# zhangyi-3/UCDIR

Hardware: AMD Instinct MI355X
Metric: restored images/sec at 50-step p_sample_loop, 256x256 SID (higher is better)
Workload: dtype bf16

## Files before the change

### ucdir_amd/csrc/conv_sk.hip.h

```cpp
#pragma once
#include "conv_halo.hip.h"
#include "akgm_ws.hip.h"

struct ConvSkP {
    const bf16_t* A; long long a_par_stride;
    const bf16_t* B0; const bf16_t* B1; int c0, ld0, ld1;
    int nchunks;
    int nb, H, W, Wp, Hp;
    int ns, Ws, Wpe, HpWpe, npos;
    float inv_per_b, inv_HpWpe, inv_Wpe;
    int ntiles, rowtiles, npar;
    int nhp;
    int nfeat;
    float alpha; int fold; int act;
    const stat_t* stats0; const stat_t* stats1; double inv_count;
    const float* bias; const float* Tb; const float* Tg; int tab_ld;
    const bf16_t* res; int res_ld;
    bf16_t* out; int out_ld;
    stat_t* stats_out;
    int units, ndp;
    float* partial;
    int alt_units; const bf16_t* alt_A; const float* alt_bias; bf16_t* alt_out; int alt_out_ld;
    int mix_wt, mix_nt, mix_nhp, mix_nunits, mix_nndp, mix_q0, mix_srt;
    unsigned long long* dbg;
};

template <int MW, int NW = 8>
struct CvSk {
    static constexpr int NWN = NW / MW;
    static constexpr int NPX = 64 * NWN;
    static constexpr int ROWS = 128 * MW;
    static constexpr int STAGE = 8192 * MW;
    static constexpr int PW = 8 * MW / NW;
    static constexpr bool LDS_TAB = NW == 8;
    static constexpr int OFF_W = 0;
    static constexpr int OFF_TB = 4 * STAGE;
    static constexpr int OFF_TG = OFF_TB + (LDS_TAB ? 9 * ROWS * 4 : 0);
    static constexpr int OFF_MS = OFF_TG + (LDS_TAB ? 9 * ROWS * 4 : 0);
// ... 5 lines not shown
    static constexpr int LDS_MAX = NW == 8 ? 160 * 1024 : 80 * 1024;
    __host__ __device__ static constexpr int lds_bytes(int nhp) { return OFF_H + 2 * nhp * 1024; }
    __host__ __device__ static constexpr int part_floats() { return ROWS * NPX; }
};

#ifdef UCDIR_TIMING
#define SK_STAMP() do { if (dbg_on && dbg_n < 120) p.dbg[dbg_off + dbg_n++] = __builtin_amdgcn_s_memtime(); } while (0)
#else
#define SK_STAMP() do {} while (0)
#endif

__device__ __forceinline__ void sk_dma16(const void* sbase, unsigned voff, unsigned lds_dst) {
    asm volatile("s_mov_b32 m0, %2\n\ts_nop 0\n\tglobal_load_lds_dwordx4 %0, %1" :: "v"(voff), "s"(sbase), "s"(lds_dst) : "memory", "m0");
}

template <int N>
__device__ __forceinline__ void sk_wait_vm() { asm volatile("s_waitcnt vmcnt(%0)" :: "n"(N) : "memory"); }

struct SkSched {
    int units, ndp, nch, G;
    long long tc;
    __host__ __device__ SkSched(int units_, int ndp_, int nch_, int G_) : units(units_), ndp(ndp_), nch(nch_), G(G_), tc((long long)(units_ - ndp_) * nch_) {}
    __host__ __device__ long long start(int g) const { return tc * g / G; }
};

__device__ __forceinline__ int sk_udiv(int q, int d, float inv_d) {
    int t = (int)((float)q * inv_d);
    t = t * d > q ? t - 1 : t;
    t = (t + 1) * d <= q ? t + 1 : t;
    return t;
// ... 278 lines not shown
            float v[16];
#pragma unroll
            for (int g4 = 0; g4 < 4; ++g4) {
                f32x4_t bv = {0.f, 0.f, 0.f, 0.f};
                if (p.alt_bias) bv = *reinterpret_cast<const f32x4_t*>(p.alt_bias + fo + 4 * g4);
#pragma unroll
                for (int e = 0; e < 4; ++e) v[4 * g4 + e] = acc[f][n][4 * g4 + e] + bv[e];
            }
            bf16_t* op = p.alt_out + opos * p.alt_out_ld + fo;
            *reinterpret_cast<uint4*>(op) = pack8_bf16(v);
            *reinterpret_cast<uint4*>(op + 8) = pack8_bf16(v + 8);
        }
    }
}

template <int MW, int NW, int NTAPS, int NF = 4>
__device__ __forceinline__ void conv_sk_body(const ConvSkP& p, unsigned char* smem, const int lid, const int G, const int units_arg, const int ndp_arg,
                                             const int qbase, const int nhp) {
    using L = CvSk<MW, NW>;
    static_assert(NF == 4 || (NF == 2 && MW == 1 && NW == 4), "short units: four waves of 64 x 64");
    constexpr int PWN = L::PW * NF / 4;
    constexpr int RSUB = 4 / NF;
    constexpr int NWN = L::NWN;
    const int tid = threadIdx.x, lane = tid & 63, l31 = lane & 31, hh = lane >> 5;
    const int wave = __builtin_amdgcn_readfirstlane(tid >> 6);
    const int wm = wave / NWN, wn = wave % NWN;
#ifdef UCDIR_TIMING
    const bool dbg_on = p.dbg && (lid == G / 2 + 3 || lid == G - 3) && (lane == 0) && (wave == NW - 1);
    const int dbg_off = lid == G - 3 ? 128 : 0;
    int dbg_n = 0;
#endif
    SK_STAMP();
    const int Wp = p.Wpe, nch = p.nchunks;
    const int HB = nhp * 1024;
    constexpr int NHW = L::NHW;
    constexpr int TA = NTAPS - 3 > 1 ? NTAPS - 3 : 1;
    constexpr int HPER = (NHW + TA - 1) / TA;

    const unsigned a_lane = L::OFF_W + (NF == 4 ? (4 * wm) * 2048 : 0) + lane * 16;
    unsigned bx[NTAPS];
    auto set_bx = [&](int py, int pxp) {
#pragma unroll
        for (int t = 0; t < NTAPS; ++t) {
            int ky, kx;
            if (NTAPS == 9) { ky = t / 3; kx = t - 3 * ky; } else { ky = py + (t >> 1); kx = pxp + (t & 1); }
            const int hp = wn * 64 + l31 + ky * Wp + kx;
            bx[t] = L::OFF_H + (hp << 6) + (((hh ^ (hp >> 2)) & 3) << 4);
        }
    };
    if (NTAPS == 9) set_bx(0, 0);
    const int hpos0 = (lane >> 2) - Wp - 1;
    const unsigned hsw = (unsigned)(((lane & 3) ^ ((lane >> 4) & 3)) << 3);
    auto piece_of = [&](int j) { const int i = j * NW + wave; return i < nhp ? i : nhp - 1; };

    const SkSched sch(units_arg, ndp_arg, nch, G);
    const long long c_beg = sch.start(lid), c_end = sch.start(lid + 1);
    const int ndp_mine = lid < ndp_arg ? (ndp_arg - lid + G - 1) / G : 0;
    long long cpos = c_beg;
    int dpi = 0;
    struct Seg { int unit, cb, ce, par, rt, tile; bool first_sk, ok; };
// ... 25 lines not shown
        const bool first = ch < p.c0;
        const int ld = first ? p.ld0 : p.ld1;
        hsrc = first ? p.B0 + ch : p.B1 + (ch - p.c0);
        if (ld != ld_cur) {
#pragma unroll
            for (int j = 0; j < NHW; ++j) hq[j] = ((((hq[j] >> 1) - hsw) / (unsigned)ld_cur) * (unsigned)ld + hsw) * 2u;
            ld_cur = ld;
        }
    };
    const unsigned char* a_seg = nullptr;
    const unsigned lane16 = (unsigned)lane * 16u;
    int seg_cb = 0;
    auto issue_halo = [&](int j, int buf) {
        sk_dma16(hsrc, hq[j], (unsigned)(L::OFF_H + piece_of(j) * 1024 + buf * HB));
    };
    auto issue_stage = [&](int k, int slot) {
#pragma unroll
        for (int j = 0; j < PWN; ++j)
            sk_dma16(a_seg + (long long)k * L::STAGE + j * 1024, lane16, (unsigned)(L::OFF_W + slot * L::STAGE + (wave * PWN + j) * 1024));
    };
    constexpr int NTP = 10;
    auto issue_table = [&](int rt, int i, int buf) {
        const int seg = 2 * i + (lane >> 5);
        const float* src = reinterpret_cast<const float*>(p.A);
        if (seg == 0 || seg > 18) { if (p.bias) src = p.bias + rt * L::ROWS; }
        else if (seg < 10) { if (p.fold) src = p.Tb + (long long)(seg - 1) * p.tab_ld + rt * L::ROWS; }
        else if (p.fold) src = p.Tg + (long long)(seg - 10) * p.tab_ld + rt * L::ROWS;
        __builtin_amdgcn_global_load_lds((const GLOBAL_AS void*)(src + (lane & 31) * 4), (LDS_AS void*)(smem + L::OFF_H + buf * HB + i * 1024), 16, 0, 0);
    };
    int hb0 = 0;
    auto prefetch = [&](const Seg& s) {
        if (NTAPS != 9) set_bx(s.par >> 1, s.par & 1);
        const int q0 = qbase + s.tile * L::NPX;
#pragma unroll
        for (int j = 0; j < NHW; ++j) {
            int q = q0 + hpos0 + 16 * piece_of(j);
            q = q < 0 ? 0 : (q >= p.npos ? (q - p.npos < p.npos ? q - p.npos : 0) : q);
            int b, yp, xs, xp;
            sk_decode(p, q, b, yp, xs, xp);
            xp = xp < p.Wp ? xp : p.Wp - 1;
            hq[j] = (unsigned)((b * p.Hp + yp) * p.Wp + xp);
        }
        ld_cur = s.cb * 32 < p.c0 ? p.ld0 : p.ld1;
#pragma unroll
        for (int j = 0; j < NHW; ++j) hq[j] = (hq[j] * (unsigned)ld_cur + hsw) * 2u;
        halo_chunk(s.cb);
        a_seg = reinterpret_cast<const unsigned char*>(p.A + (long long)s.par * p.a_par_stride + ((long long)(s.rt / RSUB) * nch * NTAPS) * (L::STAGE / 2) +
                                                       (s.rt % RSUB) * (L::STAGE / 2 / RSUB) + (wave * PWN) * 512);
        seg_cb = s.cb;
#pragma unroll
        for (int j = 0; j < NHW; ++j) issue_halo(j, hb0);
#pragma unroll
        for (int k = 0; k < 4; ++k) issue_stage(s.cb * NTAPS + k, k);
    };

    Seg cur = next_segment();
    if (!cur.ok) return;
    int rt_cur = cur.rt;
    prefetch(cur);
    auto sample_range = [&](const Seg& s) {
        const int per_b = p.ns * p.HpWpe;
        const int b0 = sk_udiv(qbase + s.tile * L::NPX, per_b, p.inv_per_b);
        int b1 = sk_udiv(qbase + s.tile * L::NPX + L::NPX - 1, per_b, p.inv_per_b) + 1; b1 = b1 < p.nb ? b1 : p.nb;
        if (b0 < b1) sk_sample_table(p, reinterpret_cast<float*>(smem + L::OFF_MS) + 2 * b0, b0, b1, wave, NW, lane);
    };
    if (L::LDS_TAB) {
// ... 31 lines not shown
            const unsigned b0 = (bx[t] + boff) ^ (jj << 5);
            lds_read16_asm<0>(fb[jj][0], b0);
            lds_read16_asm<2048>(fb[jj][1], b0);
        };
        __builtin_amdgcn_sched_barrier(0);
        unsigned bcur = hb0 ? (unsigned)HB : 0u;
        reads(std::integral_constant<int, 0>{}, std::integral_constant<int, 0>{}, 0, bcur);
        reads(std::integral_constant<int, 0>{}, std::integral_constant<int, 1>{}, 0, bcur);

        int h = 0;
        const bool want_tab = !L::LDS_TAB && cb == 0 && ce == nch;
#pragma unroll 1
        for (int c = cb; c < ce; ++c) {
            const unsigned bnext = bcur ? 0u : (unsigned)HB;
            const int cn = c + 1 < ce ? c + 1 : c;
            halo_chunk(cn);
            static_for<0, NTAPS>([&](auto tc) {
                constexpr int t = decltype(tc)::value;
                constexpr int tn = (t + 1) % NTAPS;
                constexpr int tm1 = (t + NTAPS - 1) % NTAPS;
                const unsigned boffn = tn == 0 ? bnext : bcur;
                const unsigned aan = a_lane + (unsigned)(((h + 1) & 3) * L::STAGE);
                auto unit = [&](auto jc, auto&& shadow) {
                    constexpr int jj = decltype(jc)::value;
                    const unsigned b0 = (bx[tn] + boffn) ^ (jj << 5);
#define SK_MF(f, n) acc[f][n] = __builtin_amdgcn_mfma_f32_32x32x16_bf16(fa[jj][f], fb[jj][n], acc[f][n], 0, 0, 0); __builtin_amdgcn_sched_barrier(0)
                    if constexpr (NF == 2) {
                        SK_MF(0, 0); shadow(std::integral_constant<int, 0>{}); __builtin_amdgcn_sched_barrier(0);
                        SK_MF(1, 0); lds_read16_asm<0>(fb[jj][0], b0); shadow(std::integral_constant<int, 1>{}); __builtin_amdgcn_sched_barrier(0);
                        SK_MF(0, 1); lds_read16_asm<0 * 2048 + jj * 1024>(fa[jj][0], aan); shadow(std::integral_constant<int, 2>{}); __builtin_amdgcn_sched_barrier(0);
                        SK_MF(1, 1); lds_read16_asm<1 * 2048 + jj * 1024>(fa[jj][1], aan); lds_read16_asm<2048>(fb[jj][1], b0); __builtin_amdgcn_sched_barrier(0);
                    } else {
                    SK_MF(0, 0); shadow(std::integral_constant<int, 0>{}); __builtin_amdgcn_sched_barrier(0);
                    SK_MF(1, 0); shadow(std::integral_constant<int, 1>{}); __builtin_amdgcn_sched_barrier(0);
                    SK_MF(2, 0); shadow(std::integral_constant<int, 2>{}); __builtin_amdgcn_sched_barrier(0);
#ifdef SK_ABL_NOREAD
// ... 7 lines not shown
#endif
                    }
#undef SK_MF
                };
#ifndef SK_ABL_NOREAD
                lgkm_wait_asm<NF + 2>();
#endif
                unit(std::integral_constant<int, 0>{}, [&](auto) {});
#ifndef SK_ABL_NOREAD
                lgkm_wait_asm<NF + 2>();
#endif
                {
                    constexpr int j0p = tm1 * HPER < NHW ? tm1 * HPER : NHW, j1p = (tm1 + 1) * HPER < NHW ? (tm1 + 1) * HPER : NHW;
                    constexpr int c1 = tm1 < TA ? j1p - j0p : 0;
#ifndef SK_ABL_NODMA
                    sk_wait_vm<PWN + c1>();
#endif
#ifndef SK_ABL_NOBAR
                    asm volatile("s_barrier" ::: "memory");
#endif
                }
                unit(std::integral_constant<int, 1>{}, [&](auto sc) {
                    constexpr int sidx = decltype(sc)::value;
                    constexpr int j0 = t < TA ? (t * HPER < NHW ? t * HPER : NHW) : 0, j1 = t < TA ? ((t + 1) * HPER < NHW ? (t + 1) * HPER : NHW) : 0;
                    constexpr int nh = j1 - j0;
                    constexpr int total = nh + PWN;
                    static_for<0, total>([&](auto qc) {
                        constexpr int q = decltype(qc)::value;
#ifdef SK_ABL_NODMA
                        constexpr int sh = 99;
#else
                        constexpr int sh = q * 3 / total;
#endif
                        if constexpr (sh == sidx) {
                            if constexpr (q < nh) {
                                constexpr int j = j0 + q;
                                if (want_tab && c + 1 == ce && j * NW + wave < NTP) issue_table(cur.rt / RSUB, j * NW + wave, bnext ? 1 : 0);
                                else issue_halo(j, bnext ? 1 : 0);
                            } else {
                                constexpr int j = q - nh;
                                sk_dma16(a_seg + (long long)(cb * NTAPS + h + 4) * L::STAGE + j * 1024, lane16, (unsigned)(L::OFF_W + (h & 3) * L::STAGE + (wave * PWN + j) * 1024));
                            }
                        }
                    });
                });
                ++h;
            });
            bcur = bnext;
        }
        asm volatile("s_waitcnt vmcnt(0) lgkmcnt(0)" ::: "memory");
#pragma unroll
        for (int jj = 0; jj < 2; ++jj) {
#pragma unroll
            for (int f = 0; f < NF; ++f) asm volatile("" : "+v"(fa[jj][f]));
            asm volatile("" : "+v"(fb[jj][0]), "+v"(fb[jj][1]));
        }
        __builtin_amdgcn_sched_barrier(0);
        asm volatile("s_barrier" ::: "memory");
        SK_STAMP();
        const bool same_rt = nxt.ok && (nxt.rt == rt_cur || !L::LDS_TAB);
        const unsigned tab_base = (unsigned)L::OFF_H + bcur;
        hb0 = bcur ? 0 : 1;
        if (same_rt) prefetch(nxt);
        __builtin_amdgcn_sched_barrier(0);

        if (NF != 4 || (cb == 0 && ce == nch)) {
            sk_epilogue<MW, NW, L::LDS_TAB ? 1 : 2, true, NF>(p, smem, nullptr, acc, cur.par, cur.rt / RSUB, qbase + cur.tile * L::NPX, wm, wn, lane, tab_base, -1,
                                                             (cur.rt % RSUB) * (32 * NF));
        } else if constexpr (NF == 4) {
            float* pw = p.partial + ((long long)(2 * lid + (cur.first_sk ? 0 : 1))) * L::part_floats() + wave * (128 * 64) + lane * 4;
#pragma unroll
            for (int f = 0; f < 4; ++f)
#pragma unroll
                for (int n = 0; n < 2; ++n)
#pragma unroll
// ... 40 lines not shown
        }
        if (!mixed) {
            const int q = nblk >> 3, r = nblk & 7, xcd = bid & 7;
            lid = (xcd < r ? xcd * (q + 1) : r * (q + 1) + (xcd - r) * q) + (bid >> 3);
            G = nblk;
        }
        if (MW == 1 && NW == 4) {
            if (alt) {
                const int lane = threadIdx.x & 63, wave = __builtin_amdgcn_readfirstlane(threadIdx.x >> 6);
                sk_alt_unit<NW>(p, smem, lid, wave, lane);
                return;
            }
        }
    }
    conv_sk_body<MW, NW, NTAPS>(p, smem, lid, G, p.units, p.ndp, 0, p.nhp);
}

template <int MW, int NW>
__global__ __launch_bounds__(64) void conv_sk_finish_kernel(const ConvSkP p, int G) {
    using L = CvSk<MW, NW>;
    __shared__ float ms[2 * L::MAXB];
    constexpr int NWN = L::NWN;
    const int lane = threadIdx.x;
    const int wave = blockIdx.x >> 2, fsel = blockIdx.x & 3;
    const int wm = wave / NWN, wn = wave % NWN;
    const int nch = p.nchunks;
    const SkSched sch(p.units, p.ndp, nch, G);
    const int u = blockIdx.y;
    const long long a = (long long)u * nch, b = a + nch;
    int g = (int)(a * G / sch.tc);
// ... 64 lines not shown
```

### ucdir_amd/csrc/engine.hip

```cpp
#include <hip/hip_runtime.h>

#include <cmath>
#include <cstdio>
#include <cstring>
#include <map>
#include <mutex>
#include <set>
#include <array>
#include <atomic>
#include <memory>
#include <string>
#include <vector>

#include "../../include/ucdir_hip.h"
#include "cgemm.hip.h"
#include "conv_halo.hip.h"
#include "akgm_halo.hip.h"
#include "akgm_pre.hip.h"
#include "akgm_ws.hip.h"
#include "akgm_ws32.hip.h"
#include "akgm_ws64.hip.h"
#include "conv_ws.hip.h"
#include "conv_sk.hip.h"
#include "conv_ws128.hip.h"
// ... 62 lines not shown
    ~DevPool() { release(); }
};

struct ConvW {
    bf16_t* A = nullptr; float* bias = nullptr; float* Tb = nullptr; float* Tg = nullptr;
    int rows_pad = 0, Kpad = 0, ntaps = 0, cin = 0, cout = 0, TM = 128; bool fold = false;
    bf16_t* Aup = nullptr; int Kup = 0;
    bf16_t* A10 = nullptr; float* bias_res = nullptr;
    bf16_t* Aws = nullptr;
    bf16_t* Aws128 = nullptr;
    bf16_t* Aqkv = nullptr;
    bf16_t* Atile = nullptr;
    bf16_t* Ask[2] = {nullptr, nullptr}; bf16_t* Ask_up[2] = {nullptr, nullptr};
    long long sk_up_stride[2] = {0, 0};
    bf16_t* Ask1x1 = nullptr;
};
struct AkgmW {
    bf16_t* A = nullptr; float* bias = nullptr; float* Tb = nullptr; float* Tg = nullptr;
    float* Tbb = nullptr;
    bf16_t* Apre = nullptr;
    bf16_t* Aws32 = nullptr;
    bf16_t* Aws64 = nullptr;
    int C = 0, cg = 0, Kpad = 0;
};

static int pick_tm(int cout) { return cout >= 128 ? 128 : 64; }

static ConvW upload_conv(DevPool& pool, const float* w, const float* bias, const float* gamma, const float* beta,
                         int cout, int cin, int ks) {
    ConvW W;
    W.TM = pick_tm(cout);
    PackedConv P = pack_conv(w, bias, gamma, beta, cout, cin, ks, W.TM);
    W.A = pool.upload(P.A); W.bias = pool.upload(P.bias);
    W.fold = gamma != nullptr;
    if (W.fold) { W.Tb = pool.upload(P.Tb); W.Tg = pool.upload(P.Tg); }
    W.rows_pad = P.rows_pad; W.Kpad = P.Kpad; W.ntaps = P.ntaps; W.cin = cin; W.cout = cout;
    if (ks == 3 && cin == 64 && cout == 64 && P.Kpad == 576) W.Aws = pool.upload(pack_conv_ws(P));
    if (ks == 3 && cin % 32 == 0 && P.Kpad == 9 * cin && P.rows_pad % W.TM == 0) W.Atile = pool.upload(pack_conv_tiled(P, W.TM));
    if (ks == 3 && cin % 32 == 0 && P.Kpad == 9 * cin && cout % 128 == 0) {
        W.Ask[0] = pool.upload(pack_conv_sk(P.A, 1, P.rows_pad, P.Kpad, cin, 9, 1));
        if (cout % 256 == 0) W.Ask[1] = pool.upload(pack_conv_sk(P.A, 1, P.rows_pad, P.Kpad, cin, 9, 2));
    }
    if (ks == 1 && cin % 32 == 0 && P.Kpad == cin && cout % 128 == 0 && gamma == nullptr) W.Ask1x1 = pool.upload(pack_conv_sk(P.A, 1, P.rows_pad, P.Kpad, cin, 1, 1));
    if (ks == 1 && cout == 3 * cin && gamma != nullptr && (cin == 256 || cin == 512) && P.Kpad == cin && P.rows_pad >= cout) W.Aqkv = pool.upload(pack_qkv_ws(P, cin));
    return W;
}
static void upload_upconv(DevPool& pool, ConvW& W, const float* w, const float* bias) {
    PackedConv P = pack_upconv(w, bias, W.cout, W.cin, W.TM);
    W.Aup = pool.upload(P.A); W.Kup = P.Kpad;
    for (int mw = 1; mw <= 2; ++mw)
        if (W.cin % 32 == 0 && W.cout % (128 * mw) == 0) {
            std::vector<bf16_t> img = pack_conv_sk(P.A, 4, P.rows_pad, P.Kpad, W.cin, 4, mw);
            W.sk_up_stride[mw - 1] = (long long)((img.size() - (size_t)4 * 4 * mw * 2 * 512) / 4);
            W.Ask_up[mw - 1] = pool.upload(img);
        }
}
static AkgmW upload_akgm(DevPool& pool, const float* wsp, const float* bsp, const float* gamma, const float* beta, int C) {
// ... 60 lines not shown
    set_lds_attr(conv3x3_halo_kernel<64, false>, hc_lds_bytes<64>());
    set_lds_attr(conv3x3_halo_kernel<64, true>, hc_lds_bytes<64>());
    set_lds_attr(akgm_halo_stage_kernel, AH_LDS); set_lds_attr(akgm_halo_kernel<true>, AH_LDS);
    set_lds_attr(akgm_pre_kernel<8>, AkPre<8>::LDS);
    set_lds_attr(akgm_ws_kernel<8>, AkWs::LDS); set_lds_attr(akgm_ws_kernel<16>, AkWs::LDS);
    set_lds_attr(akgm_ws32_kernel<32>, AkWs32::LDS); set_lds_attr(akgm_ws32_kernel<16>, AkWs32::LDS); set_lds_attr(akgm_ws32_kernel<8>, AkWs32::LDS);
    set_lds_attr(akgm_ws64_kernel<2, 4>, 160 * 1024); set_lds_attr(akgm_ws64_kernel<4, 4>, 160 * 1024);
    set_lds_attr(akgm_ws64_kernel<2, 8>, 160 * 1024); set_lds_attr(akgm_ws64_kernel<4, 8>, 160 * 1024);
    set_lds_attr(akgm_ws64_kernel<2, 8, true>, 160 * 1024); set_lds_attr(akgm_ws64_kernel<4, 8, true>, 160 * 1024);
    set_lds_attr(qkv_ws_kernel<256>, QkvWs::LDS); set_lds_attr(qkv_ws_kernel<512>, QkvWs::LDS);
    set_lds_attr(conv_ws_kernel, CvWs::LDS);
    set_lds_attr(conv_ws128_kernel, CvWs128::LDS);
    set_lds_attr(conv_sk_kernel<2, 8, 9>, 160 * 1024); set_lds_attr(conv_sk_kernel<2, 8, 4>, 160 * 1024);
    set_lds_attr(conv_sk_kernel<1, 8, 9>, 160 * 1024); set_lds_attr(conv_sk_kernel<1, 8, 4>, 160 * 1024);
    set_lds_attr(conv_sk_kernel<1, 4, 9>, 80 * 1024, true); set_lds_attr(conv_sk_kernel<1, 4, 4>, 80 * 1024, true);

    set_lds_attr(final_conv_kernel, 160 * 1024);
    set_lds_attr(flash_attn_kernel<1, false>, fa_lds_bytes(128)); set_lds_attr(flash_attn_kernel<1, true>, fa_lds_bytes(128));
    set_lds_attr(flash_attn_kernel<2, false>, fa_lds_bytes(256)); set_lds_attr(flash_attn_kernel<2, true>, fa_lds_bytes(256));
    set_lds_attr(flash_attn_kernel<3, false>, fa_lds_bytes(384)); set_lds_attr(flash_attn_kernel<3, true>, fa_lds_bytes(384));
    set_lds_attr(flash_attn_kernel<4, false>, fa_lds_bytes(512)); set_lds_attr(flash_attn_kernel<4, true>, fa_lds_bytes(512));
    set_lds_attr(flash_attn2_kernel<1, false>, fa_lds_bytes(128), true); set_lds_attr(flash_attn2_kernel<1, true>, fa_lds_bytes(128), true);
    set_lds_attr(flash_attn2_kernel<2, false>, fa_lds_bytes(256), true); set_lds_attr(flash_attn2_kernel<2, true>, fa_lds_bytes(256), true);
    set_lds_attr(flash_attn2_kernel<3, false>, fa_lds_bytes(384), true); set_lds_attr(flash_attn2_kernel<3, true>, fa_lds_bytes(384), true);
    set_lds_attr(flash_attn2_kernel<4, false>, fa_lds_bytes(512), true); set_lds_attr(flash_attn2_kernel<4, true>, fa_lds_bytes(512), true);
    done.insert(dev);
}

static void gemm_work(const GemmP& p, int epi, double& flops, double& bytes) {
    const double cols = ((p.cols_mode == COLS_PLAIN) ? (double)p.W : (double)p.H * p.W) * (p.up_phase ? 4.0 : 1.0);
// ... 340 lines not shown
    return true;
}
static bool try_conv_sk(const ConvW& w, const Act& x0, const Act* x1, Act& y, bool upph, int act, const Act* res, bool want_stats, hipStream_t st, bool* did_res, Act* res_out, const ConvW* wres) {
    static const bool env_on = !getenv("UCDIR_NO_CONV_SK");
    static const int env_kind = getenv("UCDIR_CONV_SK_MODE") ? atoi(getenv("UCDIR_CONV_SK_MODE")) : 2;
    const int mode = g_convsk.load();
    if (mode == 0 || (mode < 0 && !env_on)) return false;
    if (x0.C % 32 || (x1 && x1->C % 32) || y.C % 8) return false;
    const int kind = mode > 0 ? mode : env_kind;
    const int fm = mode > 0 ? 1 : -1;
    if (kind == 2) return try_conv_sk_mw<1, 4>(w, x0, x1, y, upph, act, res, want_stats, st, fm, did_res, res_out, wres);
    if (w.cout % 256 == 0) return try_conv_sk_mw<2, 8>(w, x0, x1, y, upph, act, res, want_stats, st, fm, did_res, nullptr, nullptr);
    return try_conv_sk_mw<1, 8>(w, x0, x1, y, upph, act, res, want_stats, st, fm, did_res, nullptr, nullptr);
}

static bool run_conv(const ConvW& w, const Act& x0, const Act* x1, Act& y, int mode, int act, const Act* res,
                     bool want_stats, hipStream_t st, float* nchw_out = nullptr, int crop_h = 0, int crop_w = 0,
                     Act* res_out = nullptr, const ConvW* wres = nullptr) {
    GemmP p; zero_gemm(p);
    const int cin = x0.C + (x1 ? x1->C : 0);
    require(cin == w.cin, "run_conv: channel mismatch");
    require(y.C == w.cout, "run_conv: cout mismatch");
    p.A = w.A; p.a_ld = w.Kpad; p.a_rows = w.rows_pad;
    p.B0 = x0.p; p.b0_bstride = x0.bstride(); p.ld0 = x0.C; p.c0 = x0.C;
    if (x1) { p.B1 = x1->p; p.b1_bstride = x1->bstride(); p.ld1 = x1->C; }
    p.cols_mode = mode;
    p.H = y.H; p.W = y.W; p.Wp = y.W + 2;
    p.Hi = x0.H; p.Wi = x0.W; p.Wpi = x0.W + 2;
    p.p0 = p.Wp + 1; p.pn = (y.H - 1) * p.Wp + y.W;
    p.ntaps = w.ntaps; p.cg = cin; p.cpt = cin / 8; p.cpt_shift = 0;
// ... 15 lines not shown
    const bool halo = upph || (g_use_halo && mode == COLS_S1 && w.ntaps == 9 && x0.C % 64 == 0 && (!x1 || x1->C % 64 == 0));
    if (halo) {
        const int gh = upph ? x0.H : y.H, gw = upph ? x0.W : y.W;
        choose_tile(gh, gw, p.th, p.tw);
        p.tiles_x = (gw + p.tw - 1) / p.tw; p.tiles_y = (gh + p.th - 1) / p.th;
        p.tiles = p.tiles_x * p.tiles_y;
        if (upph) {
            p.up_phase = 1; p.A = w.Aup; p.a_ld = w.Kup; p.a_gstride = (long long)w.rows_pad * w.Kup;
            p.H = x0.H; p.W = x0.W; p.Wp = x0.W + 2;
            p.tiles *= 4;
        }
    }
    if (want_stats) {
        p.stats_out = y.stats;
    }
    if (halo && !nchw_out) {
        bool sk_res = false;
        static const bool sk_tail = !getenv("UCDIR_NO_TAIL_RES");
        if (try_conv_sk(w, x0, x1, y, upph, act, res, want_stats, st, &sk_res, sk_tail ? res_out : nullptr, wres)) return sk_res;
    }
#ifdef UCDIR_TIMING
    static unsigned long long* dbgbuf = nullptr;
    if (!dbgbuf) HIPC(hipMalloc((void**)&dbgbuf, 256 * 8));
    HIPC(hipMemset(dbgbuf, 0, 256 * 8));
    p.dbg = dbgbuf;
#endif
    int tm_run = w.TM;
    if (halo && tm_run == 128 && p.nbatch * p.tiles * p.rowtiles < 256) {
        tm_run = 64; p.rowtiles = w.rows_pad / 64;
    }
// ... 623 lines not shown
    std::vector<float> tw;
    int nb = 0;
    for (size_t li = 0; li < c->layers.size(); ++li) {
        const LayerDesc& d = c->layers[li];
        LayerW& w = c->lw[li];
        if (d.kind == "stem") {
            const auto& sw = W_(c, d.name + ".weight", (size_t)d.cout * d.cin * 9);
            require(d.cin == 6, "stem expects in_channel == 6 (cat[cond, x_t])");
            std::vector<float> t((size_t)54 * d.cout);
            for (int o = 0; o < d.cout; ++o) for (int ci = 0; ci < 6; ++ci) for (int k = 0; k < 9; ++k)
                t[(size_t)(k * 6 + ci) * d.cout + o] = sw[((size_t)o * 6 + ci) * 9 + k];
            require(d.cout % 64 == 0, "stem: inner_channel must be a multiple of 64");
            w.stem_w = c->wpool.upload(pack_stem_frags(t, W_(c, d.name + ".bias", (size_t)d.cout), 6, d.cout));
        } else if (d.kind == "down" || d.kind == "up") {
            w.conv = upload_conv(c->wpool, W_(c, d.name + ".conv.weight", (size_t)d.cout * d.cin * 9).data(),
                                 W_(c, d.name + ".conv.bias", d.cout).data(), nullptr, nullptr, d.cout, d.cin, 3);
            if (d.kind == "up") upload_upconv(c->wpool, w.conv, W_(c, d.name + ".conv.weight", (size_t)d.cout * d.cin * 9).data(),
                                              W_(c, d.name + ".conv.bias", d.cout).data());
        } else {
            const std::string r = d.name + ".res_block.";
            w.block_index = nb++;
            w.conv = upload_conv(c->wpool, W_(c, r + "conv1.weight", (size_t)d.cout * d.cin * 9).data(),
                                 W_(c, r + "conv1.bias", d.cout).data(), W_(c, r + "norm1.weight", d.cin).data(),
                                 W_(c, r + "norm1.bias", d.cin).data(), d.cout, d.cin, 3);
            w.has_res = d.cin != d.cout;
            if (w.has_res) {
                w.resconv = upload_conv(c->wpool, W_(c, r + "res_conv.weight", (size_t)d.cout * d.cin).data(),
                                        W_(c, r + "res_conv.bias", d.cout).data(), nullptr, nullptr, d.cout, d.cin, 1);
                if (w.conv.TM == 64 && d.cin % 64 == 0 && w.conv.Kpad == 9 * d.cin) {
                    PackedConv P = pack_conv(W_(c, r + "conv1.weight", (size_t)d.cout * d.cin * 9).data(), nullptr,
                                             W_(c, r + "norm1.weight", d.cin).data(), W_(c, r + "norm1.bias", d.cin).data(),
// ... 582 lines not shown

int32_t ucdir_op_conv(const float* x0, int32_t c0, const float* x1, int32_t c1, int32_t B, int32_t H, int32_t W,
                      const float* w_host, const float* bias_host, const float* gamma_host, const float* beta_host,
                      int32_t cout, int32_t ksize, int32_t mode, int32_t silu, const float* residual, float* y,
                      double* stats_out_host, void* stream) {
    API_BEGIN
    ensure_kernel_attrs();
    hipStream_t st = (hipStream_t)stream;
    DevPool pool;
    Act a0 = act_from_nchw(pool, x0, B, c0, H, W, st, true);
    Act a1; if (x1) a1 = act_from_nchw(pool, x1, B, c1, H, W, st, true);
    int Ho = H, Wo = W;
    if (mode == COLS_DOWN) { Ho = H / 2; Wo = W / 2; } else if (mode == COLS_UP) { Ho = 2 * H; Wo = 2 * W; }
    Act out = make_act(pool, B, Ho, Wo, cout);
    Act res; if (residual) res = act_from_nchw(pool, residual, B, cout, Ho, Wo, st, false);
    ConvW w = upload_conv(pool, w_host, bias_host, gamma_host, beta_host, cout, c0 + (x1 ? c1 : 0), ksize);
    if (mode == COLS_UP && ksize == 3) upload_upconv(pool, w, w_host, bias_host);
    run_conv(w, a0, x1 ? &a1 : nullptr, out, mode, silu, residual ? &res : nullptr, true, st);
    hipLaunchKernelGGL(act_to_nchw_kernel, dim3(2048), dim3(256), 0, st, out.p, y, B, cout, Ho, Wo);
    HIPC(hipGetLastError());
    std::vector<stat_t> sfx;
    if (stats_out_host) { sfx.resize((size_t)2 * UCDIR_STAT_SLOTS * B); HIPC(hipMemcpyAsync(sfx.data(), out.stats, sizeof(stat_t) * sfx.size(), hipMemcpyDeviceToHost, st)); }
    HIPC(hipStreamSynchronize(st));
    if (stats_out_host)
        for (int bb = 0; bb < B; ++bb)
            for (int q = 0; q < 2; ++q) {
                stat_t acc = 0;
                for (int k = 0; k < UCDIR_STAT_SLOTS; ++k) acc += sfx[((size_t)bb * UCDIR_STAT_SLOTS + k) * 2 + q];
                stats_out_host[bb * 2 + q] = (double)acc / UCDIR_STAT_SCALE;
            }
    API_END
// ... 312 lines not shown
```

### ucdir_amd/csrc/pack.h

```cpp
#pragma once
#include <cmath>
#include <cstdint>
#include <vector>

#include "common.h"

struct PackedConv {
    std::vector<bf16_t> A;
    std::vector<float> bias;
    std::vector<float> Tb, Tg;
    int rows_pad = 0, Kpad = 0, ntaps = 0, cin = 0, cout = 0, ncls = 0;
};

static inline bool tap_valid(int cls, int tap) {
    const int cy = cls / 3, cx = cls % 3, ky = tap / 3, kx = tap % 3;
    if (cy == 0 && ky == 0) return false;
    if (cy == 2 && ky == 2) return false;
    if (cx == 0 && kx == 0) return false;
    if (cx == 2 && kx == 2) return false;
    return true;
}

static inline PackedConv pack_conv(const float* w, const float* bias, const float* gamma, const float* beta,
                                   int cout, int cin, int ks, int TM) {
// ... 172 lines not shown
    for (int rt = 0; rt < nrt; ++rt)
        for (int c = 0; c < nch; ++c)
            for (int u = 0; u < nsteps; ++u)
                for (int k = 0; k < 16; ++k)
                    for (int lane = 0; lane < 64; ++lane) {
                        const int row = (k % ipt) * 16 + (lane >> 2);
                        int tap = TPS * u + k / ipt; tap = tap < 9 ? tap : 8;
                        const int lc = (lane & 3) ^ ((row >> 2) & 3);
                        const bf16_t* src = &P.A[(size_t)(rt * TM + row) * P.Kpad + (size_t)tap * P.cin + c * 32 + lc * 8];
                        bf16_t* dst = &img[((((size_t)rt * nch + c) * nsteps + u) * 16 + k) * 512 + lane * 8];
                        for (int e = 0; e < 8; ++e) dst[e] = src[e];
                    }
    return img;
}

static inline std::vector<bf16_t> pack_conv_sk(const std::vector<bf16_t>& A, int npar, int rows_pad, int Kld, int cin, int ntaps, int MW) {
    const int ROWS = 128 * MW, nrt = (rows_pad + ROWS - 1) / ROWS, nch = cin / 32, nf = 4 * MW;
    std::vector<bf16_t> img((size_t)npar * nrt * nch * ntaps * nf * 2 * 512 + (size_t)4 * nf * 2 * 512, 0);
    for (int par = 0; par < npar; ++par)
        for (int rt = 0; rt < nrt; ++rt)
            for (int c = 0; c < nch; ++c)
                for (int t = 0; t < ntaps; ++t)
                    for (int f = 0; f < nf; ++f)
                        for (int j = 0; j < 2; ++j)
                            for (int lane = 0; lane < 64; ++lane) {
                                const int rho = lane & 31, hh = lane >> 5;
                                const int row = rt * ROWS + 32 * f + 16 * ((rho >> 2) & 1) + (rho & 3) + 4 * (rho >> 3);
                                if (row >= rows_pad) continue;
                                const bf16_t* src = &A[((size_t)par * rows_pad + row) * Kld + (size_t)t * cin + 32 * c + 16 * j + 8 * hh];
                                bf16_t* dst = &img[(((((((size_t)par * nrt + rt) * nch + c) * ntaps + t) * nf + f) * 2 + j) * 64 + lane) * 8];
                                for (int e = 0; e < 8; ++e) dst[e] = src[e];
                            }
    return img;
}

static inline std::vector<bf16_t> pack_akgm_ws32(const float* wsp, const float* gamma, int C) {
    const int cg = C / 8, nk = (cg == 32) ? 18 : ((cg == 16) ? 9 : 5), nb = C / 32;
    std::vector<bf16_t> img((size_t)nb * 8 * nk * 2 * 32 * 8, 0);
    for (int blk = 0; blk < nb; ++blk)
        for (int w = 0; w < 8; ++w)
            for (int rho = 0; rho < 32; ++rho) {
                const int c4 = 2 * ((rho >> 2) & 1) + (rho >> 4), sm = 4 * ((rho >> 3) & 1) + (rho & 3);
                const int c = 32 * blk + 4 * w + c4, o = 8 * c + sm, g = c / cg;
                for (int j = 0; j < nk; ++j)
// ... 82 lines not shown
```

Measured before the change: 37.24.

## Add stride-2 downsample path to stream-K halo conv kernel with parity planes

Adds a dedicated stride-2 (downsample) variant of the stream-K halo convolution. It loads the input as four parity planes into LDS via conditional DMA, reorders taps so that each plane's halo load overlaps the MFMA sub-steps, and packs the weights in a matching tap order. Downsample convs previously went through the generic path. This reuses the halo/LDS pipeline for them, in exchange for extra complexity, a disabled same-row-tile prefetch, and new correctness risk in the plane indexing.

After: 37.27 (median of 6 runs). No clear change (+0.1%).

```diff
diff --git a/ucdir_amd/csrc/conv_sk.hip.h b/ucdir_amd/csrc/conv_sk.hip.h
--- a/ucdir_amd/csrc/conv_sk.hip.h
+++ b/ucdir_amd/csrc/conv_sk.hip.h
@@ -22,6 +22,8 @@
     float* partial;
     int alt_units; const bf16_t* alt_A; const float* alt_bias; bf16_t* alt_out; int alt_out_ld;
     int mix_wt, mix_nt, mix_nhp, mix_nunits, mix_nndp, mix_q0, mix_srt;
+    int dn_Hp, dn_Wp;
+    int dn_np[4];
     unsigned long long* dbg;
 };
 
@@ -57,6 +59,11 @@
     asm volatile("s_mov_b32 m0, %2\n\ts_nop 0\n\tglobal_load_lds_dwordx4 %0, %1" :: "v"(voff), "s"(sbase), "s"(lds_dst) : "memory", "m0");
 }
 
+__device__ __forceinline__ void sk_dma16_if(const void* sbase, unsigned voff, unsigned lds_dst, int idx, int lim) {
+    asm volatile("s_cmp_lt_i32 %3, %4\n\ts_cbranch_scc0 1f\n\ts_mov_b32 m0, %2\n\ts_nop 0\n\tglobal_load_lds_dwordx4 %0, %1\n1:"
+                 :: "v"(voff), "s"(sbase), "s"(lds_dst), "s"(idx), "s"(lim) : "memory", "m0", "scc");
+}
+
 template <int N>
 __device__ __forceinline__ void sk_wait_vm() { asm volatile("s_waitcnt vmcnt(%0)" :: "n"(N) : "memory"); }
 
@@ -365,11 +372,14 @@
     }
 }
 
-template <int MW, int NW, int NTAPS, int NF = 4>
+template <int T> struct DnTap { static constexpr bool Y = T == 2 || T == 5 || T == 6; };
+
+template <int MW, int NW, int NTAPS, int NF = 4, bool DOWN = false>
 __device__ __forceinline__ void conv_sk_body(const ConvSkP& p, unsigned char* smem, const int lid, const int G, const int units_arg, const int ndp_arg,
                                              const int qbase, const int nhp) {
     using L = CvSk<MW, NW>;
     static_assert(NF == 4 || (NF == 2 && MW == 1 && NW == 4), "short units: four waves of 64 x 64");
+    static_assert(!DOWN || (NTAPS == 9 && NF == 4 && MW == 1 && NW == 4), "stride 2: the one-shot 4-wave frame, one 9-sub-step cycle per chunk");
     constexpr int PWN = L::PW * NF / 4;
     constexpr int RSUB = 4 / NF;
     constexpr int NWN = L::NWN;
@@ -394,7 +404,9 @@
 #pragma unroll
         for (int t = 0; t < NTAPS; ++t) {
             int ky, kx;
-            if (NTAPS == 9) { ky = t / 3; kx = t - 3 * ky; } else { ky = py + (t >> 1); kx = pxp + (t & 1); }
+            if (DOWN) {
+                ky = t == 3 || t == 4 || t == 6; kx = t == 1 || t == 4 || t == 8;
+            } else if (NTAPS == 9) { ky = t / 3; kx = t - 3 * ky; } else { ky = py + (t >> 1); kx = pxp + (t & 1); }
             const int hp = wn * 64 + l31 + ky * Wp + kx;
             bx[t] = L::OFF_H + (hp << 6) + (((hh ^ (hp >> 2)) & 3) << 4);
         }
@@ -450,6 +462,10 @@
     auto issue_halo = [&](int j, int buf) {
         sk_dma16(hsrc, hq[j], (unsigned)(L::OFF_H + piece_of(j) * 1024 + buf * HB));
     };
+    auto plane_off = [&](int pl) { return (long long)((pl >> 1) * p.dn_Wp + (pl & 1)) * p.ld0; };
+    auto dn_halo = [&](const bf16_t* src, int j, int pl, unsigned buf_off) {
+        sk_dma16_if(src, hq[j], (unsigned)(L::OFF_H + piece_of(j) * 1024) + buf_off, j * NW + wave, p.dn_np[pl]);
+    };
     auto issue_stage = [&](int k, int slot) {
 #pragma unroll
         for (int j = 0; j < PWN; ++j)
@@ -475,7 +491,7 @@
             int b, yp, xs, xp;
             sk_decode(p, q, b, yp, xs, xp);
             xp = xp < p.Wp ? xp : p.Wp - 1;
-            hq[j] = (unsigned)((b * p.Hp + yp) * p.Wp + xp);
+            hq[j] = DOWN ? (unsigned)((b * p.dn_Hp + 2 * yp) * p.dn_Wp + 2 * xp) : (unsigned)((b * p.Hp + yp) * p.Wp + xp);
         }
         ld_cur = s.cb * 32 < p.c0 ? p.ld0 : p.ld1;
 #pragma unroll
@@ -485,7 +501,14 @@
                                                        (s.rt % RSUB) * (L::STAGE / 2 / RSUB) + (wave * PWN) * 512);
         seg_cb = s.cb;
 #pragma unroll
-        for (int j = 0; j < NHW; ++j) issue_halo(j, hb0);
+        for (int j = 0; j < NHW; ++j) {
+            if (DOWN) dn_halo(hsrc, j, 0, (unsigned)(hb0 * HB));
+            else issue_halo(j, hb0);
+        }
+        if (DOWN) {
+#pragma unroll
+            for (int j = 0; j < NHW; ++j) dn_halo(hsrc + plane_off(3), j, 3, (unsigned)((1 - hb0) * HB));
+        }
 #pragma unroll
         for (int k = 0; k < 4; ++k) issue_stage(s.cb * NTAPS + k, k);
     };
@@ -547,12 +570,13 @@
         for (int c = cb; c < ce; ++c) {
             const unsigned bnext = bcur ? 0u : (unsigned)HB;
             const int cn = c + 1 < ce ? c + 1 : c;
+            const bf16_t* const hsrc_c = p.B0 + c * 32;
             halo_chunk(cn);
             static_for<0, NTAPS>([&](auto tc) {
                 constexpr int t = decltype(tc)::value;
                 constexpr int tn = (t + 1) % NTAPS;
                 constexpr int tm1 = (t + NTAPS - 1) % NTAPS;
-                const unsigned boffn = tn == 0 ? bnext : bcur;
+                const unsigned boffn = (tn == 0 || (DOWN && DnTap<tn>::Y)) ? bnext : bcur;
                 const unsigned aan = a_lane + (unsigned)(((h + 1) & 3) * L::STAGE);
                 auto unit = [&](auto jc, auto&& shadow) {
                     constexpr int jj = decltype(jc)::value;
@@ -590,15 +614,19 @@
                     constexpr int j0p = tm1 * HPER < NHW ? tm1 * HPER : NHW, j1p = (tm1 + 1) * HPER < NHW ? (tm1 + 1) * HPER : NHW;
                     constexpr int c1 = tm1 < TA ? j1p - j0p : 0;
 #ifndef SK_ABL_NODMA
-                    sk_wait_vm<PWN + c1>();
+                    if constexpr (DOWN) sk_wait_vm<PWN>();
+                    else sk_wait_vm<PWN + c1>();
 #endif
 #ifndef SK_ABL_NOBAR
                     asm volatile("s_barrier" ::: "memory");
 #endif
+                    if constexpr (DOWN) SK_STAMP();
                 }
                 unit(std::integral_constant<int, 1>{}, [&](auto sc) {
                     constexpr int sidx = decltype(sc)::value;
-                    constexpr int j0 = t < TA ? (t * HPER < NHW ? t * HPER : NHW) : 0, j1 = t < TA ? ((t + 1) * HPER < NHW ? (t + 1) * HPER : NHW) : 0;
+                    constexpr bool dnh = DOWN && (t == 2 || t == 4 || t == 6 || t == 8);
+                    constexpr int j0 = DOWN ? 0 : (t < TA ? (t * HPER < NHW ? t * HPER : NHW) : 0);
+                    constexpr int j1 = DOWN ? (dnh ? NHW : 0) : (t < TA ? ((t + 1) * HPER < NHW ? (t + 1) * HPER : NHW) : 0);
                     constexpr int nh = j1 - j0;
                     constexpr int total = nh + PWN;
                     static_for<0, total>([&](auto qc) {
@@ -611,7 +639,14 @@
                         if constexpr (sh == sidx) {
                             if constexpr (q < nh) {
                                 constexpr int j = j0 + q;
-                                if (want_tab && c + 1 == ce && j * NW + wave < NTP) issue_table(cur.rt / RSUB, j * NW + wave, bnext ? 1 : 0);
+                                if constexpr (DOWN) {
+                                    constexpr int pl = t == 2 ? 1 : (t == 4 ? 2 : (t == 6 ? 0 : 3));
+                                    constexpr bool toY = t == 2 || t == 6;
+                                    const unsigned hbuf = toY ? bnext : bcur;
+                                    const bf16_t* const src = (t <= 4 ? hsrc_c : hsrc) + plane_off(pl);
+                                    if (t == 6 && want_tab && c + 1 == ce && j * NW + wave < NTP) issue_table(cur.rt / RSUB, j * NW + wave, bnext ? 1 : 0);
+                                    else dn_halo(src, j, pl, hbuf);
+                                } else if (want_tab && c + 1 == ce && j * NW + wave < NTP) issue_table(cur.rt / RSUB, j * NW + wave, bnext ? 1 : 0);
                                 else issue_halo(j, bnext ? 1 : 0);
                             } else {
                                 constexpr int j = q - nh;
@@ -634,7 +669,7 @@
         __builtin_amdgcn_sched_barrier(0);
         asm volatile("s_barrier" ::: "memory");
         SK_STAMP();
-        const bool same_rt = nxt.ok && (nxt.rt == rt_cur || !L::LDS_TAB);
+        const bool same_rt = nxt.ok && (nxt.rt == rt_cur || !L::LDS_TAB) && !DOWN;
         const unsigned tab_base = (unsigned)L::OFF_H + bcur;
         hb0 = bcur ? 0 : 1;
         if (same_rt) prefetch(nxt);
@@ -705,6 +740,14 @@
         }
     }
     conv_sk_body<MW, NW, NTAPS>(p, smem, lid, G, p.units, p.ndp, 0, p.nhp);
+}
+
+__global__ __launch_bounds__(256, 2) void conv_sk_down_kernel(const ConvSkP p) {
+    extern __shared__ __attribute__((aligned(16))) unsigned char smem[];
+    const int nblk = gridDim.x, bid = blockIdx.x;
+    const int q = nblk >> 3, r = nblk & 7, xcd = bid & 7;
+    const int lid = (xcd < r ? xcd * (q + 1) : r * (q + 1) + (xcd - r) * q) + (bid >> 3);
+    conv_sk_body<1, 4, 9, 4, true>(p, smem, lid, nblk, p.units, p.ndp, 0, p.nhp);
 }
 
 template <int MW, int NW>
diff --git a/ucdir_amd/csrc/engine.hip b/ucdir_amd/csrc/engine.hip
--- a/ucdir_amd/csrc/engine.hip
+++ b/ucdir_amd/csrc/engine.hip
@@ -100,6 +100,7 @@
     bf16_t* Ask[2] = {nullptr, nullptr}; bf16_t* Ask_up[2] = {nullptr, nullptr};
     long long sk_up_stride[2] = {0, 0};
     bf16_t* Ask1x1 = nullptr;
+    bf16_t* Ask_dn = nullptr;
 };
 struct AkgmW {
     bf16_t* A = nullptr; float* bias = nullptr; float* Tb = nullptr; float* Tg = nullptr;
@@ -113,7 +114,7 @@
 static int pick_tm(int cout) { return cout >= 128 ? 128 : 64; }
 
 static ConvW upload_conv(DevPool& pool, const float* w, const float* bias, const float* gamma, const float* beta,
-                         int cout, int cin, int ks) {
+                         int cout, int cin, int ks, bool down = false) {
     ConvW W;
     W.TM = pick_tm(cout);
     PackedConv P = pack_conv(w, bias, gamma, beta, cout, cin, ks, W.TM);
@@ -127,6 +128,8 @@
         W.Ask[0] = pool.upload(pack_conv_sk(P.A, 1, P.rows_pad, P.Kpad, cin, 9, 1));
         if (cout % 256 == 0) W.Ask[1] = pool.upload(pack_conv_sk(P.A, 1, P.rows_pad, P.Kpad, cin, 9, 2));
     }
+    if (down && ks == 3 && cin % 32 == 0 && P.Kpad == 9 * cin && cout % 128 == 0 && gamma == nullptr)
+        W.Ask_dn = pool.upload(pack_conv_sk(P.A, 1, P.rows_pad, P.Kpad, cin, 9, 1, CONV_SK_DN_TAPS));
     if (ks == 1 && cin % 32 == 0 && P.Kpad == cin && cout % 128 == 0 && gamma == nullptr) W.Ask1x1 = pool.upload(pack_conv_sk(P.A, 1, P.rows_pad, P.Kpad, cin, 1, 1));
     if (ks == 1 && cout == 3 * cin && gamma != nullptr && (cin == 256 || cin == 512) && P.Kpad == cin && P.rows_pad >= cout) W.Aqkv = pool.upload(pack_qkv_ws(P, cin));
     return W;
@@ -217,6 +220,7 @@
     set_lds_attr(conv_sk_kernel<2, 8, 9>, 160 * 1024); set_lds_attr(conv_sk_kernel<2, 8, 4>, 160 * 1024);
     set_lds_attr(conv_sk_kernel<1, 8, 9>, 160 * 1024); set_lds_attr(conv_sk_kernel<1, 8, 4>, 160 * 1024);
     set_lds_attr(conv_sk_kernel<1, 4, 9>, 80 * 1024, true); set_lds_attr(conv_sk_kernel<1, 4, 4>, 80 * 1024, true);
+    set_lds_attr(conv_sk_down_kernel, 80 * 1024, true);
 
     set_lds_attr(final_conv_kernel, 160 * 1024);
     set_lds_attr(flash_attn_kernel<1, false>, fa_lds_bytes(128)); set_lds_attr(flash_attn_kernel<1, true>, fa_lds_bytes(128));
@@ -587,6 +591,86 @@
     return try_conv_sk_mw<1, 8>(w, x0, x1, y, upph, act, res, want_stats, st, fm, did_res, nullptr, nullptr);
 }
 
+static bool try_conv_sk_down(const ConvW& w, const Act& x0, Act& y, bool want_stats, hipStream_t st) {
+    using L = CvSk<1, 4>;
+    static const bool env_on = !getenv("UCDIR_NO_SK_DOWN");
+    const int mode = g_convsk.load();
+    if (mode == 0 || mode == 1 || (mode < 0 && !env_on) || !w.Ask_dn) return false;
+    const int cin = x0.C, Hi = x0.H, Wi = x0.W, B = x0.B;
+    if (cin % 32 || y.C % 8 || (Hi & 1) || (Wi & 1) || y.H != Hi / 2 || y.W != Wi / 2 || B > L::MAXB) return false;
+    const int H = y.H, W = y.W, Wpe = W + 1, HpWpe = (H + 1) * Wpe;
+    const int NPX = L::NPX;
+    const int nhp = (NPX + Wpe + 1 + 15) / 16;
+    if (nhp > L::NHP_MAX || L::lds_bytes(nhp) > L::LDS_MAX) return false;
+    const long long npos = (long long)B * HpWpe;
+    if ((long long)B * (Hi + 2) * (Wi + 2) * (long long)(cin > y.C ? cin : y.C) >= (1LL << 31) || npos >= (1LL << 30)) return false;
+    ConvSkP p; std::memset(&p, 0, sizeof(p));
+    p.A = w.Ask_dn;
+    p.B0 = x0.p; p.ld0 = x0.C; p.c0 = x0.C;
+    p.nchunks = cin / 32;
+    p.nb = B; p.H = H; p.W = W; p.Wp = W + 2; p.Hp = H + 2;
+    p.dn_Hp = Hi + 2; p.dn_Wp = Wi + 2;
+    for (int pl = 0; pl < 4; ++pl) p.dn_np[pl] = (NPX + (pl == 0 ? Wpe + 1 : (pl == 1 ? Wpe : (pl == 2 ? 1 : 0))) + 15) / 16;
+    p.ns = 1; p.Ws = W; p.Wpe = Wpe; p.HpWpe = HpWpe; p.npos = (int)npos;
+    p.inv_per_b = 1.0f / (float)HpWpe; p.inv_HpWpe = 1.0f / (float)HpWpe; p.inv_Wpe = 1.0f / (float)Wpe;
+    p.ntiles = (int)((npos + NPX - 1) / NPX); p.rowtiles = (w.cout + L::ROWS - 1) / L::ROWS; p.npar = 1;
+    p.nhp = nhp; p.nfeat = w.cout;
+    p.alpha = 1.f; p.fold = 0; p.act = 0;
+    p.bias = w.bias;
+    p.out = y.p; p.out_ld = y.C;
+    if (want_stats) p.stats_out = y.stats;
+    p.units = p.rowtiles * p.ntiles;
+    int G = p.units; p.ndp = p.units;
+    const int ncu = num_cus();
+    if (g_persist_grid > 0) {
+        G = g_persist_grid < p.units ? (int)g_persist_grid : p.units; if (G > SK_MAX_GRID) G = SK_MAX_GRID; p.ndp = (p.units / G) * G;
+        const long long rem = (long long)p.units - p.ndp;
+        if (rem > 0 && rem * p.nchunks < G && p.ndp >= G) p.ndp -= G;
+    } else if (p.units >= 64 && p.units < ncu && p.nchunks >= 16) {
+        G = 2 * p.units; p.ndp = 0;
+    } else if (mode < 0 && (p.units < ncu || p.nchunks < 4)) return false;
+    const size_t lds = L::lds_bytes(nhp);
+    const int nsk = p.units - p.ndp;
+    p.partial = nsk > 0 ? splitk_scratch() : nullptr;
+    auto go = [&]() {
+        hipLaunchKernelGGL(conv_sk_down_kernel, dim3(G), dim3(L::THREADS), lds, st, p);
+        if (nsk > 0) hipLaunchKernelGGL((conv_sk_finish_kernel<1, 4>), dim3(4 * 4, nsk), dim3(64), 0, st, p, G);
+    };
+#ifdef UCDIR_TIMING
+    {
+        static unsigned long long* dbgbuf = nullptr;
+        if (!dbgbuf) HIPC(hipMalloc((void**)&dbgbuf, 256 * 8));
+        HIPC(hipMemset(dbgbuf, 0, 256 * 8));
+        p.dbg = dbgbuf;
+        go();
+        unsigned long long h[256];
+        HIPC(hipStreamSynchronize(st));
+        HIPC(hipMemcpy(h, dbgbuf, sizeof(h), hipMemcpyDeviceToHost));
+        for (int w2 = 0; w2 < 2; ++w2) {
+            const int n = (int)h[255 - w2];
+            fprintf(stderr, "CONV_SK_DOWN TIMING %s units=%d grid=%d n=%d: start %llu |", w2 ? "last-round" : "first-round", p.units, G, n, h[128 * w2] - (h[0] < h[128] ? h[0] : h[128]));
+            for (int i = 1; i < n && i < 120; ++i) fprintf(stderr, " %llu", h[128 * w2 + i] - h[128 * w2 + i - 1]);
+            fprintf(stderr, "\n");
+        }
+        return true;
+    }
+#endif
+    if (g_prof.on) {
+        ProfEntry e; e.key = 132;
+        const double cols = (double)H * W * B;
+        e.flops = 2.0 * 9 * cin * (double)w.cout * cols;
+        e.bytes = (double)cin * Hi * Wi * 2 * B + (double)w.cout * cols * 2 + 9.0 * cin * w.cout * 2;
+        e.dH = H; e.dW = W; e.dCin = 9 * cin; e.dCout = w.cout;
+        e.e0 = g_prof.get(); e.e1 = g_prof.get();
+        HIPC(hipEventRecord(e.e0, st));
+        go();
+        HIPC(hipEventRecord(e.e1, st));
+        g_prof.entries.push_back(e);
+    } else go();
+    HIPC(hipGetLastError());
+    return true;
+}
+
 static bool run_conv(const ConvW& w, const Act& x0, const Act* x1, Act& y, int mode, int act, const Act* res,
                      bool want_stats, hipStream_t st, float* nchw_out = nullptr, int crop_h = 0, int crop_w = 0,
                      Act* res_out = nullptr, const ConvW* wres = nullptr) {
@@ -632,6 +716,7 @@
     if (want_stats) {
         p.stats_out = y.stats;
     }
+    if (mode == COLS_DOWN && !x1 && !res && act == 0 && !nchw_out && !w.fold && try_conv_sk_down(w, x0, y, want_stats, st)) return false;
     if (halo && !nchw_out) {
         bool sk_res = false;
         static const bool sk_tail = !getenv("UCDIR_NO_TAIL_RES");
@@ -1285,7 +1370,7 @@
             w.stem_w = c->wpool.upload(pack_stem_frags(t, W_(c, d.name + ".bias", (size_t)d.cout), 6, d.cout));
         } else if (d.kind == "down" || d.kind == "up") {
             w.conv = upload_conv(c->wpool, W_(c, d.name + ".conv.weight", (size_t)d.cout * d.cin * 9).data(),
-                                 W_(c, d.name + ".conv.bias", d.cout).data(), nullptr, nullptr, d.cout, d.cin, 3);
+                                 W_(c, d.name + ".conv.bias", d.cout).data(), nullptr, nullptr, d.cout, d.cin, 3, d.kind == "down");
             if (d.kind == "up") upload_upconv(c->wpool, w.conv, W_(c, d.name + ".conv.weight", (size_t)d.cout * d.cin * 9).data(),
                                               W_(c, d.name + ".conv.bias", d.cout).data());
         } else {
@@ -1898,7 +1983,7 @@
     if (mode == COLS_DOWN) { Ho = H / 2; Wo = W / 2; } else if (mode == COLS_UP) { Ho = 2 * H; Wo = 2 * W; }
     Act out = make_act(pool, B, Ho, Wo, cout);
     Act res; if (residual) res = act_from_nchw(pool, residual, B, cout, Ho, Wo, st, false);
-    ConvW w = upload_conv(pool, w_host, bias_host, gamma_host, beta_host, cout, c0 + (x1 ? c1 : 0), ksize);
+    ConvW w = upload_conv(pool, w_host, bias_host, gamma_host, beta_host, cout, c0 + (x1 ? c1 : 0), ksize, mode == COLS_DOWN);
     if (mode == COLS_UP && ksize == 3) upload_upconv(pool, w, w_host, bias_host);
     run_conv(w, a0, x1 ? &a1 : nullptr, out, mode, silu, residual ? &res : nullptr, true, st);
     hipLaunchKernelGGL(act_to_nchw_kernel, dim3(2048), dim3(256), 0, st, out.p, y, B, cout, Ho, Wo);
diff --git a/ucdir_amd/csrc/pack.h b/ucdir_amd/csrc/pack.h
--- a/ucdir_amd/csrc/pack.h
+++ b/ucdir_amd/csrc/pack.h
@@ -210,7 +210,9 @@
     return img;
 }
 
-static inline std::vector<bf16_t> pack_conv_sk(const std::vector<bf16_t>& A, int npar, int rows_pad, int Kld, int cin, int ntaps, int MW) {
+static constexpr int CONV_SK_DN_TAPS[9] = {0, 2, 4, 6, 8, 1, 7, 3, 5};
+static inline std::vector<bf16_t> pack_conv_sk(const std::vector<bf16_t>& A, int npar, int rows_pad, int Kld, int cin, int ntaps, int MW,
+                                               const int* tap_order = nullptr) {
     const int ROWS = 128 * MW, nrt = (rows_pad + ROWS - 1) / ROWS, nch = cin / 32, nf = 4 * MW;
     std::vector<bf16_t> img((size_t)npar * nrt * nch * ntaps * nf * 2 * 512 + (size_t)4 * nf * 2 * 512, 0);
     for (int par = 0; par < npar; ++par)
@@ -223,7 +225,8 @@
                                 const int rho = lane & 31, hh = lane >> 5;
                                 const int row = rt * ROWS + 32 * f + 16 * ((rho >> 2) & 1) + (rho & 3) + 4 * (rho >> 3);
                                 if (row >= rows_pad) continue;
-                                const bf16_t* src = &A[((size_t)par * rows_pad + row) * Kld + (size_t)t * cin + 32 * c + 16 * j + 8 * hh];
+                                const int ts = tap_order ? tap_order[t] : t;
+                                const bf16_t* src = &A[((size_t)par * rows_pad + row) * Kld + (size_t)ts * cin + 32 * c + 16 * j + 8 * hh];
                                 bf16_t* dst = &img[(((((((size_t)par * nrt + rt) * nch + c) * ntaps + t) * nf + f) * 2 + j) * 64 + lane) * 8];
                                 for (int e = 0; e < 8; ++e) dst[e] = src[e];
                             }
```
